# senli1073/SeisT

Measured on NVIDIA H100. Metric: waveforms/sec (B,3,8192) seist_m_dpk fwd+bwd, higher is better.
Workload: dtype f32

## Files before the change

### seist_b200/csrc/api.cu

```cuda
#include <atomic>
#include <cstdio>
#include <cstdlib>
#include <cstring>
#include <vector>
#include "common.cuh"

namespace seist {

static thread_local char g_err[512] = "";
static std::atomic<uint64_t> g_launches{0};
static int g_sm_count = 0;

void set_error(const char* msg) {
  std::strncpy(g_err, msg, sizeof(g_err) - 1);
  g_err[sizeof(g_err) - 1] = 0;
}
void note_launch() { g_launches.fetch_add(1, std::memory_order_relaxed); }
int check_launch(const char* what) {
  cudaError_t e = cudaPeekAtLastError();
  if (e != cudaSuccess) {
    cudaGetLastError();
    std::snprintf(g_err, sizeof(g_err), "%s: %s", what, cudaGetErrorString(e));
    return (int)e;
  }
  return 0;
}

int launch_conv_fwd(const SeistOp& op, cudaStream_t s);
int launch_conv_bwd_data(const SeistOp& op, cudaStream_t s);
int launch_conv_bwd_w(const SeistOp& op, cudaStream_t s, int sm_count);
int launch_res_bwd(const SeistOp& op, cudaStream_t s);
int launch_att_fwd(const SeistOp& op, cudaStream_t s);
int launch_att_bwd_q(const SeistOp& op, cudaStream_t s);
int launch_att_bwd_kv(const SeistOp& op, cudaStream_t s);
int launch_headvec_fwd(const SeistOp& op, cudaStream_t s);
int launch_headvec_bwd(const SeistOp& op, cudaStream_t s);
int launch_bn_finalize(const SeistOp& op, bool fwd, cudaStream_t s);
bool pw_eligible(const SeistOp& op);
int launch_pw_fwd(const SeistOp& op, cudaStream_t s, int sm_count);
int launch_pw_bwd_data(const SeistOp& op, cudaStream_t s, int sm_count);
int launch_res_bwd4(const SeistOp& op, cudaStream_t s, int sm_count);
bool bww_eligible(const SeistOp& op);
int launch_bww_any(const SeistOp& op, cudaStream_t s, int sm_count);
bool convk_eligible(const SeistOp& op);
bool bwwk_eligible(const SeistOp& op);
bool convk_bwd_data_eligible(const SeistOp& op);
int launch_bwwk(const SeistOp& op, cudaStream_t s, int sm_count);
int launch_convk_fwd(const SeistOp& op, cudaStream_t s);
int launch_convk_bwd_data(const SeistOp& op, cudaStream_t s);
int launch_bn_prepare(const SeistOp& op, bool fwd, cudaStream_t s);
int launch_stem_compose(const SeistOp& op, bool fwd, cudaStream_t s);
bool tcconv_eligible(const SeistOp& op, int mode);
int launch_tcconv(const SeistOp& op, int mode, cudaStream_t s, int sm_count);
int tcconv_error_flag();

static int tcc_mode() {
  static int v = -1;
  if (v < 0) { const char* e = std::getenv("SEIST_TCC"); v = !e ? 2 : (e[0] == '0' ? 0 : (e[0] == '1' ? 1 : 2)); }
  return v;
}
static bool tcc_auto(const SeistOp& op, int mode) {
  const int Kd = mode == 0 ? op.Cin : op.Cout;
  if (op.up_src_L > 0) return mode == 0 && Kd >= 32;
  if (op.k > 1) return mode == 0 ? (op.L_out <= 512 && Kd >= 16) : (op.L_out <= 256 && Kd >= 32);
  return mode == 0 && Kd >= 64 && op.L_out <= 256;
}
static bool use_tcc(const SeistOp& op, int mode) {
  const int m = tcc_mode();
  if (m == 0 || !tcconv_eligible(op, mode)) return false;
  return m == 1 || tcc_auto(op, mode);
}

static int sm_count() {
  if (g_sm_count == 0) {
    int dev = 0;
    cudaGetDevice(&dev);
    if (cudaDeviceGetAttribute(&g_sm_count, cudaDevAttrMultiProcessorCount, dev) != cudaSuccess || g_sm_count <= 0)
      g_sm_count = 132;
  }
  return g_sm_count;
}

static int validate_conv(const SeistOp& op) {
  if (op.groups <= 0 || op.Cin % op.groups || op.Cout % op.groups) { set_error("conv: channels not divisible by groups"); return -2; }
  if (op.k < 1 || op.stride < 1 || op.N < 1 || op.L_out < 1) { set_error("conv: bad geometry"); return -2; }
  if (op.n_in < 1 || op.n_in > SEIST_MAX_IN) { set_error("conv: bad n_in"); return -2; }
  if ((op.pool > 1 || op.up_src_L > 0) && op.n_in != 1) { set_error("conv: pool/upsample need a single input view"); return -2; }
  if (op.pool > 1 && (op.k != 1 || op.up_src_L > 0)) { set_error("conv: pool only with k=1"); return -2; }
  if (op.N > 65535) { set_error("conv: batch > 65535 per launch"); return -2; }
  return 0;
}

enum Family {
  F_NONE = 0, F_TCCONV_FWD, F_TCCONV_BWD_DATA, F_PW_FWD, F_CONVK_FWD, F_CONV_FWD, F_PW_BWD_DATA, F_CONVK_BWD_DATA,
  F_CONV_BWD_DATA, F_BWWK, F_BWW, F_CONV_BWD_W, F_RES_BWD, F_RES_BWD4, F_ATT_FWD, F_ATT_BWD_Q, F_ATT_BWD_KV, F_HEADVEC_FWD,
  F_HEADVEC_BWD, F_BN_FINALIZE_FWD, F_BN_FINALIZE_BWD, F_BN_PREPARE_FWD, F_BN_PREPARE_BWD, F_STEM_COMPOSE_FWD, F_STEM_COMPOSE_BWD,
  F_ZERO
};
static const char* kFamilyName[] = {
  "none", "tcconv_fwd(wgmma+TMA)", "tcconv_bwd_data(wgmma+TMA)", "pw_fwd(simt)", "convk_fwd(simt)",
  "conv_fwd(simt)", "pw_bwd_data(simt)", "convk_bwd_data(simt)", "conv_bwd_data(simt)", "bwwk(simt)", "bww(simt)",
  "conv_bwd_w(simt)", "res_bwd", "res_bwd4", "att_fwd", "att_bwd_q", "att_bwd_kv", "headvec_fwd", "headvec_bwd", "bn_finalize_fwd",
  "bn_finalize_bwd", "bn_prepare_fwd", "bn_prepare_bwd", "stem_compose_fwd", "stem_compose_bwd", "zero"
};

static Family choose(const SeistOp& op) {
  switch (op.kind) {
    case SEIST_OP_CONV_FWD:
      if (use_tcc(op, 0)) return F_TCCONV_FWD;
      if (pw_eligible(op)) return F_PW_FWD;
      return convk_eligible(op) ? F_CONVK_FWD : F_CONV_FWD;
    case SEIST_OP_CONV_BWD_DATA:
      if (use_tcc(op, 1)) return F_TCCONV_BWD_DATA;
      if (pw_eligible(op)) return F_PW_BWD_DATA;
      return convk_bwd_data_eligible(op) ? F_CONVK_BWD_DATA : F_CONV_BWD_DATA;
    case SEIST_OP_CONV_BWD_W:
      if (bwwk_eligible(op)) return F_BWWK;
      return bww_eligible(op) ? F_BWW : F_CONV_BWD_W;
    case SEIST_OP_RES_BWD: return (op.L_out & 3) ? F_RES_BWD : F_RES_BWD4;
    case SEIST_OP_ATT_FWD: return F_ATT_FWD;
    case SEIST_OP_ATT_BWD_Q: return F_ATT_BWD_Q;
    case SEIST_OP_ATT_BWD_KV: return F_ATT_BWD_KV;
    case SEIST_OP_HEADVEC_FWD: return F_HEADVEC_FWD;
    case SEIST_OP_HEADVEC_BWD: return F_HEADVEC_BWD;
    case SEIST_OP_BN_FINALIZE_FWD: return F_BN_FINALIZE_FWD;
    case SEIST_OP_BN_FINALIZE_BWD: return F_BN_FINALIZE_BWD;
    case SEIST_OP_BN_PREPARE_FWD: return F_BN_PREPARE_FWD;
    case SEIST_OP_BN_PREPARE_BWD: return F_BN_PREPARE_BWD;
    case SEIST_OP_STEM_COMPOSE_FWD: return F_STEM_COMPOSE_FWD;
    case SEIST_OP_STEM_COMPOSE_BWD: return F_STEM_COMPOSE_BWD;
    case SEIST_OP_ZERO: return F_ZERO;
    default: return F_NONE;
  }
}

static int run_one(const SeistOp& op, cudaStream_t s) {
  if (op.kind == SEIST_OP_CONV_FWD || op.kind == SEIST_OP_CONV_BWD_DATA || op.kind == SEIST_OP_CONV_BWD_W) {
    int v = validate_conv(op);
    if (v) return v;
  }
  switch (choose(op)) {
    case F_TCCONV_FWD: return launch_tcconv(op, 0, s, sm_count());
    case F_TCCONV_BWD_DATA: return launch_tcconv(op, 1, s, sm_count());
    case F_PW_FWD: return launch_pw_fwd(op, s, sm_count());
    case F_CONVK_FWD: return launch_convk_fwd(op, s);
    case F_CONV_FWD: return launch_conv_fwd(op, s);
    case F_PW_BWD_DATA: return launch_pw_bwd_data(op, s, sm_count());
    case F_CONVK_BWD_DATA: return launch_convk_bwd_data(op, s);
    case F_CONV_BWD_DATA: return launch_conv_bwd_data(op, s);
    case F_BWWK: return launch_bwwk(op, s, sm_count());
    case F_BWW: return launch_bww_any(op, s, sm_count());
    case F_CONV_BWD_W: return launch_conv_bwd_w(op, s, sm_count());
    case F_RES_BWD: return launch_res_bwd(op, s);
    case F_RES_BWD4: return launch_res_bwd4(op, s, sm_count());
    case F_ATT_FWD: return launch_att_fwd(op, s);
    case F_ATT_BWD_Q: return launch_att_bwd_q(op, s);
    case F_ATT_BWD_KV: return launch_att_bwd_kv(op, s);
    case F_HEADVEC_FWD: return launch_headvec_fwd(op, s);
    case F_HEADVEC_BWD: return launch_headvec_bwd(op, s);
    case F_BN_FINALIZE_FWD: return launch_bn_finalize(op, true, s);
    case F_BN_FINALIZE_BWD: return launch_bn_finalize(op, false, s);
    case F_BN_PREPARE_FWD: return launch_bn_prepare(op, true, s);
    case F_BN_PREPARE_BWD: return launch_bn_prepare(op, false, s);
    case F_STEM_COMPOSE_FWD: return launch_stem_compose(op, true, s);
    case F_STEM_COMPOSE_BWD: return launch_stem_compose(op, false, s);
    case F_ZERO: {
      cudaError_t e = cudaMemsetAsync(op.out.x, 0, op.zero_bytes, s);
      if (e != cudaSuccess) { set_error(cudaGetErrorString(e)); return (int)e; }
      return 0;
    }
    default: set_error("unknown op kind"); return -1;
  }
}

}

extern "C" {

int seist_plan_run(const SeistOp* ops, int32_t n, void* stream);
const char* seist_last_error(void);

int seist_abi_version(void) { return SEIST_ABI_VERSION; }
uint64_t seist_sizeof_op(void) { return sizeof(SeistOp); }
uint64_t seist_sizeof_bn(void) { return sizeof(SeistBN); }
const char* seist_last_error(void) { return seist::g_err; }
uint64_t seist_launch_count(void) { return seist::g_launches.load(); }
const char* seist_op_family(const SeistOp* op) { return op ? seist::kFamilyName[seist::choose(*op)] : "none"; }
int seist_tc_error_flag(void) { return seist::tcconv_error_flag(); }

static std::vector<cudaEvent_t> g_events[64];
static cudaEvent_t event_at(size_t i) {
  int dev = 0;
  cudaGetDevice(&dev);
  std::vector<cudaEvent_t>& pool = g_events[dev & 63];
  while (pool.size() <= i) {
    cudaEvent_t e = nullptr;
    if (cudaEventCreateWithFlags(&e, cudaEventDisableTiming) != cudaSuccess) return nullptr;
    pool.push_back(e);
  }
  return pool[i];
}
static int fork_join(cudaStream_t from, cudaStream_t to, size_t& ev) {
  cudaEvent_t e = event_at(ev++);
  if (e == nullptr) { seist::set_error("plan_run_lanes: cudaEventCreate failed"); return (int)cudaErrorMemoryAllocation; }
  cudaError_t r = cudaEventRecord(e, from);
  if (r == cudaSuccess) r = cudaStreamWaitEvent(to, e, 0);
  if (r != cudaSuccess) { seist::set_error(cudaGetErrorString(r)); return (int)r; }
  return 0;
}

int seist_plan_run_lanes(const SeistOp* ops, int32_t n, void* const* streams, int32_t n_streams) {
  if (ops == nullptr || n < 0 || streams == nullptr || n_streams < 1 || n_streams > 8) { seist::set_error("plan_run_lanes: bad arguments"); return -1; }
  if (n_streams == 1) return seist_plan_run(ops, n, streams[0]);
  cudaStream_t s0 = (cudaStream_t)streams[0];
  size_t ev = (size_t)n;
  for (int l = 1; l < n_streams; ++l) {
    size_t e = ev;
    const int fr = fork_join(s0, (cudaStream_t)streams[l], e);
    if (fr) return fr;
  }
  int rc = 0;
  for (int i = 0; i < n && rc == 0; ++i) {
    const SeistOp& op = ops[i];
    const int lane = op.lane < 0 ? 0 : (op.lane >= n_streams ? n_streams - 1 : op.lane);
    cudaStream_t s = (cudaStream_t)streams[lane];
    for (int w = 0; w < op.n_wait && w < 4 && rc == 0; ++w) {
      if (op.wait_ev[w] < 0 || op.wait_ev[w] >= n) { seist::set_error("plan_run_lanes: bad event id"); rc = -1; break; }
      cudaEvent_t e = event_at((size_t)op.wait_ev[w]);
      cudaError_t r = e ? cudaStreamWaitEvent(s, e, 0) : cudaErrorMemoryAllocation;
      if (r != cudaSuccess) { seist::set_error(cudaGetErrorString(r)); rc = (int)r; }
    }
    if (rc) break;
    rc = seist::run_one(op, s);
    if (rc != 0) {
      char buf[600];
      std::snprintf(buf, sizeof(buf), "op %d (kind %d): %s", i, op.kind, seist_last_error());
      seist::set_error(buf);
      break;
    }
    if (op.rec_event >= 0) {
      cudaEvent_t e = op.rec_event < n ? event_at((size_t)op.rec_event) : nullptr;
      cudaError_t r = e ? cudaEventRecord(e, s) : cudaErrorMemoryAllocation;
      if (r != cudaSuccess) { seist::set_error(cudaGetErrorString(r)); rc = (int)r; }
    }
  }
  for (int l = 1; l < n_streams; ++l) {
    size_t e = (size_t)n + 1 + (size_t)l;
    const int jr = fork_join((cudaStream_t)streams[l], s0, e);
    if (jr && !rc) rc = jr;
  }
  return rc;
}

int seist_plan_run(const SeistOp* ops, int32_t n, void* stream) {
  if (ops == nullptr || n < 0) { seist::set_error("plan_run: bad arguments"); return -1; }
  cudaStream_t s = (cudaStream_t)stream;
  for (int i = 0; i < n; ++i) {
    int rc = seist::run_one(ops[i], s);
    if (rc != 0) {
      char buf[600];
      std::snprintf(buf, sizeof(buf), "op %d (kind %d): %s", i, ops[i].kind, seist::g_err);
      seist::set_error(buf);
      return rc;
    }
  }
  return 0;
}

}
```

### seist_b200/csrc/pw.cu

```cuda
#include "common.cuh"
#include "conv_common.cuh"

namespace seist {

constexpr int PW_NT = 128;

__device__ __forceinline__ float4 ldg4(const float* p) { return __ldg(reinterpret_cast<const float4*>(p)); }
__device__ __forceinline__ float4 ld4(const float* p) { return *reinterpret_cast<const float4*>(p); }
__device__ __forceinline__ void st4(float* p, float4 v) { *reinterpret_cast<float4*>(p) = v; }

__device__ __forceinline__ float4 lds4(uint32_t a) {
  float4 v;
  asm volatile("ld.shared.v4.f32 {%0,%1,%2,%3}, [%4];" : "=f"(v.x), "=f"(v.y), "=f"(v.z), "=f"(v.w) : "r"(a));
  return v;
}

struct PwChan {
  const float* x;
  float* g;
  long long nstride;
  float sc, sh, mu, istd;
  int act, bn, bnc, accum;
};

// ... 406 lines not shown
  if constexpr (RING) {
    iobase = quad_base(0);
#pragma unroll
    for (int s = 0; s < PW_RING_S - 1; ++s) issue_step();
  }

  for (int g = 0; g < G; ++g) {
    const long long f = ((long long)blockIdx.x * G + g) * PW_NT + tid;
    const bool ok = f < NQ;
    const int n = ok ? (int)(f / LQ) : 0;
    const int l = ok ? (int)(f - (long long)n * LQ) * 4 : 0;
    const float pf = path_factor(op, seed, n) * alpha_factor(op, seed, n);
    float2 acc[CI_T / 2][4];
#pragma unroll
    for (int c = 0; c < CI_T / 2; ++c)
#pragma unroll
      for (int q = 0; q < 4; ++q) acc[c][q] = make_float2(0.f, 0.f);
    const size_t obase = ((size_t)n * op.out.Ct + op.out.c0) * (size_t)L + l;
    for (int co0 = 0; co0 < Cout4; co0 += PW_BD_CG) {
      float4 dx[PW_BD_CG], du[PW_BD_CG], xo[PW_BD_CG];
      if constexpr (RING) {
        issue_step();
        cp_async_wait<PW_RING_S - 1>();
        const uint32_t src0 = ring + cstage * PW_RING_STAGE_B;
        cstage = cstage + 1 == PW_RING_S ? 0 : cstage + 1;
#pragma unroll
        for (int j = 0; j < PW_BD_CG; ++j) {
          const uint32_t src = src0 + j * (3 * PW_NT * 16);
          dx[j] = op.out_dxd ? lds4(src) : make_float4(0.f, 0.f, 0.f, 0.f);
          du[j] = has_bn ? lds4(src + PW_NT * 16) : make_float4(0.f, 0.f, 0.f, 0.f);
          xo[j] = need_x ? lds4(src + 2 * PW_NT * 16) : make_float4(0.f, 0.f, 0.f, 0.f);
        }
      } else {
#pragma unroll
        for (int j = 0; j < PW_BD_CG; ++j) {
          const int co = min(co0 + j, Cout - 1);
          const size_t off = obase + (size_t)co * L;
          dx[j] = op.out_dxd ? ldg4(op.out_dxd + off) : make_float4(0.f, 0.f, 0.f, 0.f);
          du[j] = has_bn ? ldg4(op.out.g + off) : make_float4(0.f, 0.f, 0.f, 0.f);
          xo[j] = need_x ? ldg4(op.out.x + off) : make_float4(0.f, 0.f, 0.f, 0.f);
        }
      }
#pragma unroll
      for (int j = 0; j < PW_BD_CG; ++j) {
        const int co = co0 + j;
        const PwOut o = oc_s[co];
        float4 gv;
        gv.x = dx[j].x + fmaf(o.A, du[j].x, fmaf(o.Bx, xo[j].x, o.Cc));
        gv.y = dx[j].y + fmaf(o.A, du[j].y, fmaf(o.Bx, xo[j].y, o.Cc));
        gv.z = dx[j].z + fmaf(o.A, du[j].z, fmaf(o.Bx, xo[j].z, o.Cc));
        gv.w = dx[j].w + fmaf(o.A, du[j].w, fmaf(o.Bx, xo[j].w, o.Cc));
        if (op.out_act == SEIST_OUT_SIGMOID) {
          gv.x *= xo[j].x * (1.f - xo[j].x);
          gv.y *= xo[j].y * (1.f - xo[j].y);
          gv.z *= xo[j].z * (1.f - xo[j].z);
          gv.w *= xo[j].w * (1.f - xo[j].w);
        }
        gv.x *= pf;
        gv.y *= pf;
        gv.z *= pf;
        gv.w *= pf;
        if (F_ELEM) {
          const float4 kp = pw_keep4(op.p_elem, seed, op.seed_elem, ((uint64_t)n * Cout + min(co, Cout - 1)) * (uint64_t)L + l);
          gv.x *= kp.x;
          gv.y *= kp.y;
          gv.z *= kp.z;
          gv.w *= kp.w;
        }
        const float2* wr = reinterpret_cast<const float2*>(w_s + co * CI_T);
        const float2 gx = dup2(gv.x), gy = dup2(gv.y), gz = dup2(gv.z), gw = dup2(gv.w);
#pragma unroll
        for (int cp = 0; cp < CI_T / 2; ++cp) {
          const float2 w = wr[cp];
          acc[cp][0] = fma2(w, gx, acc[cp][0]);
          acc[cp][1] = fma2(w, gy, acc[cp][1]);
          acc[cp][2] = fma2(w, gz, acc[cp][2]);
          acc[cp][3] = fma2(w, gw, acc[cp][3]);
        }
      }
    }
    if (!ok) continue;
    if constexpr (F_POOL) {
#pragma unroll
      for (int col = 0; col < CI_T; ++col) {
        const PwChan& c = ch_s[col];
        if (c.g == nullptr) continue;
        const float2(&ap)[4] = acc[col >> 1];
        float4 gg = (col & 1) ? make_float4(ap[0].y, ap[1].y, ap[2].y, ap[3].y) : make_float4(ap[0].x, ap[1].x, ap[2].x, ap[3].x);
        {
          const long long soff = (long long)n * c.nstride + (long long)l * op.pool;
          float s1 = 0.f, s2 = 0.f;
          if (op.pool == 2) pool_route<2>(c, soff, gg, s1, s2);
          else if (op.pool == 4) pool_route<4>(c, soff, gg, s1, s2);
          else pool_route<8>(c, soff, gg, s1, s2);
          if (c.bn >= 0) {
            my_st[(2 * col) * 32] += s1;
            my_st[(2 * col + 1) * 32] += s2;
          }
        }
      }
    } else {
#pragma unroll
    for (int cb = 0; cb < CI_T; cb += PW_BD_EB) {
      float4 xv[PW_BD_EB], ov[PW_BD_EB];
#pragma unroll
      for (int u = 0; u < PW_BD_EB; ++u) {
        const PwChan& c = ch_s[cb + u];
        const long long off = (long long)n * c.nstride + l;
        const bool live = c.g != nullptr;
        const bool want_x = live && ((F_GELU && c.act == SEIST_ACT_GELU) || c.bn >= 0);
        xv[u] = want_x ? ldg4(c.x + off) : make_float4(0.f, 0.f, 0.f, 0.f);
        ov[u] = (live && c.accum) ? ld4(c.g + off) : make_float4(0.f, 0.f, 0.f, 0.f);
      }
#pragma unroll
      for (int u = 0; u < PW_BD_EB; ++u) {
        const int col = cb + u;
        const PwChan& c = ch_s[col];
        if (c.g == nullptr) continue;
        const float2(&ap)[4] = acc[col >> 1];
        float4 gg = (col & 1) ? make_float4(ap[0].y, ap[1].y, ap[2].y, ap[3].y) : make_float4(ap[0].x, ap[1].x, ap[2].x, ap[3].x);
        const float4 x = xv[u];
        if (F_GELU && c.act == SEIST_ACT_GELU) {
          const float4 d = pw_gelu_grad4(make_float4(fmaf(c.sc, x.x, c.sh), fmaf(c.sc, x.y, c.sh), fmaf(c.sc, x.z, c.sh),
                                                     fmaf(c.sc, x.w, c.sh)));
          gg.x *= d.x;
          gg.y *= d.y;
          gg.z *= d.z;
          gg.w *= d.w;
        }
        if (c.bn >= 0) {
          my_st[(2 * col) * 32] += (gg.x + gg.y) + (gg.z + gg.w);
          my_st[(2 * col + 1) * 32] += fmaf(gg.x, (x.x - c.mu) * c.istd, gg.y * ((x.y - c.mu) * c.istd)) +
                                       fmaf(gg.z, (x.z - c.mu) * c.istd, gg.w * ((x.w - c.mu) * c.istd));
        }
        gg.x += ov[u].x;
        gg.y += ov[u].y;
        gg.z += ov[u].z;
        gg.w += ov[u].w;
        st4(c.g + (long long)n * c.nstride + l, gg);
      }
    }
    }
  }
  float st[2 * CI_T];
#pragma unroll
  for (int i = 0; i < 2 * CI_T; ++i) st[i] = my_st[i * 32];
  cta_reduce_atomic<2 * CI_T>(st, red_s, [&](int i, float s) {
    const PwChan& c = ch_s[i >> 1];
    if (c.g != nullptr && c.bn >= 0) {
      const SeistBN& e = op.bn_table[c.bn];
      atomicAdd(&e.gstat_acc[(i & 1) * e.C + c.bnc], (double)s);
    }
  });
}

__global__ void __launch_bounds__(PW_NT) res_bwd4_kernel(const __grid_constant__ SeistOp op, const int G) {
  __shared__ float red_s[4 * 4];
  const int tid = threadIdx.x;
  const int co = blockIdx.y;
  const int L = op.L_out, LQ = L >> 2;
  const long long NQ = (long long)op.N * LQ;
  const uint64_t seed = load_seed(op.step_seed);
  const OutGradCoef kc = out_grad_coef(op, co);
  const bool has_bn = (op.out.bn >= 0 && op.out.g != nullptr);
  const bool need_x = has_bn || op.out_act == SEIST_OUT_SIGMOID;
  const SeistView& va = op.res_a;
  const SeistView& vb = op.res_b;
  const bool wa = va.C > 0 && va.g != nullptr, wb = vb.C > 0 && vb.g != nullptr;
  float amu = 0.f, aistd = 0.f, bmu = 0.f, bistd = 0.f;
  if (wa && va.bn >= 0) view_khat(op, va, co, amu, aistd);
  if (wb && vb.bn >= 0) view_khat(op, vb, co, bmu, bistd);
  float st[4] = {0.f, 0.f, 0.f, 0.f};
  for (int g = 0; g < G; ++g) {
    const long long f = ((long long)blockIdx.x * G + g) * PW_NT + tid;
    if (f >= NQ) break;
    const int n = (int)(f / LQ);
    const int l = (int)(f - (long long)n * LQ) * 4;
    const size_t off = ((size_t)n * op.out.Ct + op.out.c0 + co) * (size_t)L + l;
    float4 gv = op.out_dxd ? ldg4(op.out_dxd + off) : make_float4(0.f, 0.f, 0.f, 0.f);
    if (need_x) {
      const float4 x = ldg4(op.out.x + off);
      if (has_bn) {
        const float4 du = ldg4(op.out.g + off);
        gv.x += fmaf(kc.A, du.x, fmaf(kc.Bx, x.x, kc.Cc));
        gv.y += fmaf(kc.A, du.y, fmaf(kc.Bx, x.y, kc.Cc));
        gv.z += fmaf(kc.A, du.z, fmaf(kc.Bx, x.z, kc.Cc));
        gv.w += fmaf(kc.A, du.w, fmaf(kc.Bx, x.w, kc.Cc));
      }
      if (op.out_act == SEIST_OUT_SIGMOID) {
        gv.x *= x.x * (1.f - x.x);
        gv.y *= x.y * (1.f - x.y);
        gv.z *= x.z * (1.f - x.z);
        gv.w *= x.w * (1.f - x.w);
      }
    }
#pragma unroll
    for (int which = 0; which < 2; ++which) {
      const SeistView& v = which == 0 ? va : vb;
      if (!(which == 0 ? wa : wb)) continue;
      float4 gg = gv;
      if (which == 0) {
        const float af = alpha_factor(op, seed, n);
        gg.x *= af;
        gg.y *= af;
        gg.z *= af;
        gg.w *= af;
      }
      const size_t voff = ((size_t)n * v.Ct + v.c0 + co) * (size_t)L + l;
      if (v.bn >= 0) {
        const float4 x = ldg4(v.x + voff);
        const float mu = which == 0 ? amu : bmu, is = which == 0 ? aistd : bistd;
        st[2 * which] += (gg.x + gg.y) + (gg.z + gg.w);
        st[2 * which + 1] += fmaf(gg.x, (x.x - mu) * is, gg.y * ((x.y - mu) * is)) +
                             fmaf(gg.z, (x.z - mu) * is, gg.w * ((x.w - mu) * is));
      }
      float* gp = v.g + voff;
      if (v.accum) {
        const float4 old = ld4(gp);
        gg.x += old.x;
        gg.y += old.y;
        gg.z += old.z;
        gg.w += old.w;
      }
      st4(gp, gg);
    }
  }
  cta_reduce_atomic<4>(st, red_s, [&](int i, float s) {
    const SeistView& v = (i >> 1) == 0 ? va : vb;
    const bool w = (i >> 1) == 0 ? wa : wb;
    if (w && v.bn >= 0) {
      const SeistBN& e = op.bn_table[v.bn];
      atomicAdd(&e.gstat_acc[(i & 1) * e.C + v.bn_c0 + co], (double)s);
    }
  });
}

static bool pw_pooled_ok(const SeistOp& op) {
  if (op.pool != 2 && op.pool != 4 && op.pool != 8) return false;
  if (op.n_in != 1 || op.in[0].act != SEIST_ACT_NONE || op.in[0].L != op.L_out * op.pool) return false;
  return op.p_elem <= 0.f && op.res_a.C == 0 && op.res_b.C == 0;
}
bool pw_eligible(const SeistOp& op) {
  if (op.k != 1 || op.stride != 1 || op.groups != 1 || op.up_src_L > 0) return false;
  if (op.L_out & 3) return false;
  if (op.pool > 1) return pw_pooled_ok(op);
  return true;
}

static int pick_G(long long nq, int tiles_y, int sm_count) {
  long long ctas = (nq + PW_NT - 1) / PW_NT;
  int G = 1;
  while (G < 8 && (ctas / (2 * G)) * tiles_y >= 4LL * sm_count) G *= 2;
  return G;
}

template <typename K>
static int pw_set_smem(K kernel, size_t bytes) {
  if (bytes > 48 * 1024) {
    cudaError_t e = cudaFuncSetAttribute(kernel, cudaFuncAttributeMaxDynamicSharedMemorySize, (int)bytes);
    if (e != cudaSuccess) return (int)e;
  }
  return 0;
}

static bool any_gelu(const SeistOp& op) {
  for (int i = 0; i < op.n_in; ++i)
    if (op.in[i].act == SEIST_ACT_GELU) return true;
  return false;
}

template <int COT, bool E, bool R, bool Gf, bool P = false>
static int pw_fwd_go(const SeistOp& op, cudaStream_t s, dim3 grid, size_t smem, int G) {
  int rc = pw_set_smem(pw_fwd_kernel<COT, E, R, Gf, P>, smem);
  if (!rc) pw_fwd_kernel<COT, E, R, Gf, P><<<grid, PW_NT, smem, s>>>(op, G);
  return rc;
}
template <int COT>
static int pw_fwd_sel(const SeistOp& op, cudaStream_t s, dim3 grid, size_t smem, int G) {
  if (op.pool > 1) return pw_fwd_go<COT, false, false, false, true>(op, s, grid, smem, G);
  const int sel = (op.p_elem > 0.f ? 4 : 0) | ((op.res_a.C > 0 || op.res_b.C > 0) ? 2 : 0) | (any_gelu(op) ? 1 : 0);
  switch (sel) {
    case 0: return pw_fwd_go<COT, false, false, false>(op, s, grid, smem, G);
    case 1: return pw_fwd_go<COT, false, false, true>(op, s, grid, smem, G);
    case 2: return pw_fwd_go<COT, false, true, false>(op, s, grid, smem, G);
    case 3: return pw_fwd_go<COT, false, true, true>(op, s, grid, smem, G);
    case 4: return pw_fwd_go<COT, true, false, false>(op, s, grid, smem, G);
    case 5: return pw_fwd_go<COT, true, false, true>(op, s, grid, smem, G);
    case 6: return pw_fwd_go<COT, true, true, false>(op, s, grid, smem, G);
    default: return pw_fwd_go<COT, true, true, true>(op, s, grid, smem, G);
  }
}

int launch_pw_fwd(const SeistOp& op, cudaStream_t s, int sm_count) {
  const int cot = op.Cout > 8 ? 16 : 8;
  const int Cin8 = (op.Cin + 7) & ~7;
  const size_t smem = sizeof(PwChan) * Cin8 + sizeof(float) * ((size_t)Cin8 * cot + 5 * cot + 4 * 2 * cot + 4 * 2 * cot * 32);
  const long long nq = (long long)op.N * (op.L_out >> 2);
  const int ty = (op.Cout + cot - 1) / cot;
  const int G = pick_G(nq, ty, sm_count);
  dim3 grid((unsigned)((nq + (long long)PW_NT * G - 1) / ((long long)PW_NT * G)), ty);
  const int rc = cot == 16 ? pw_fwd_sel<16>(op, s, grid, smem, G) : pw_fwd_sel<8>(op, s, grid, smem, G);
  if (rc) return rc;
  note_launch();
  return check_launch("pw_fwd");
}

template <int CIT, bool E, bool Gf, bool P = false>
static int pw_bwdd_go(const SeistOp& op, cudaStream_t s, dim3 grid, size_t smem, int G) {
  if (!P) smem += (size_t)PW_RING_S * PW_RING_STAGE_B;
  int rc = pw_set_smem(pw_bwd_data_kernel<CIT, E, Gf, P>, smem);
  if (!rc) pw_bwd_data_kernel<CIT, E, Gf, P><<<grid, PW_NT, smem, s>>>(op, G);
  return rc;
}
template <int CIT>
static int pw_bwdd_sel(const SeistOp& op, cudaStream_t s, dim3 grid, size_t smem, int G) {
  if (op.pool > 1) return pw_bwdd_go<CIT, false, false, true>(op, s, grid, smem, G);
  const int sel = (op.p_elem > 0.f ? 2 : 0) | (any_gelu(op) ? 1 : 0);
  switch (sel) {
    case 0: return pw_bwdd_go<CIT, false, false>(op, s, grid, smem, G);
    case 1: return pw_bwdd_go<CIT, false, true>(op, s, grid, smem, G);
    case 2: return pw_bwdd_go<CIT, true, false>(op, s, grid, smem, G);
    default: return pw_bwdd_go<CIT, true, true>(op, s, grid, smem, G);
  }
}

int launch_pw_bwd_data(const SeistOp& op, cudaStream_t s, int sm_count) {
  const int cit = op.Cin > 8 ? 16 : 8;
  const int Cout4 = (op.Cout + 3) & ~3;
  const size_t smem = sizeof(PwChan) * cit + sizeof(PwOut) * Cout4 + sizeof(float) * ((size_t)Cout4 * cit + 4 * 2 * cit + 4 * 2 * cit * 32);
  const long long nq = (long long)op.N * (op.L_out >> 2);
  const int ty = (op.Cin + cit - 1) / cit;
  const int G = pick_G(nq, ty, sm_count);
  dim3 grid((unsigned)((nq + (long long)PW_NT * G - 1) / ((long long)PW_NT * G)), ty);
  const int rc = cit == 16 ? pw_bwdd_sel<16>(op, s, grid, smem, G) : pw_bwdd_sel<8>(op, s, grid, smem, G);
  if (rc) return rc;
  note_launch();
  return check_launch("pw_bwd_data");
}

int launch_res_bwd4(const SeistOp& op, cudaStream_t s, int sm_count) {
  const long long nq = (long long)op.N * (op.L_out >> 2);
  const int G = pick_G(nq, op.Cout, sm_count);
  dim3 grid((unsigned)((nq + (long long)PW_NT * G - 1) / ((long long)PW_NT * G)), op.Cout);
  res_bwd4_kernel<<<grid, PW_NT, 0, s>>>(op, G);
  note_launch();
  return check_launch("res_bwd4");
}

constexpr int BW_NT = 256;

template <int CO_B, int R_B, bool K1, int BW_PC>
__global__ void __launch_bounds__(BW_NT, 3) bww_kernel(const __grid_constant__ SeistOp op, const int nci_max, const int g_async, const int gx_off) {
  constexpr int BW_PITCH = BW_PC + 4;
  constexpr int BW_GP = 2 * BW_PC + 8;
  extern __shared__ __align__(16) unsigned char sm_raw[];
  constexpr int TGM = CO_B / 4, TGN = R_B / 8, TG = TGM * TGN, PG = BW_NT / TG;
  static_assert(TG <= BW_NT && BW_NT % TG == 0, "bad tile");
  const int k = op.k, S = op.stride, L = op.L_out;
  const int gs_in = op.Cin / op.groups, gs_out = op.Cout / op.groups;
  const int tpg = (gs_out + CO_B - 1) / CO_B;
  const int grp = blockIdx.y / tpg;
  const int Cin = (grp + 1) * gs_in;
  const int Cout = (grp + 1) * gs_out;
  const int R = gs_in * k;
  const int width = BW_PC * S + k - S;
  const int pitch = K1 ? BW_PITCH : (width | 1);
  const int stage_f = (CO_B / 2) * BW_GP + nci_max * pitch;
  const int area_f = stage_f > BW_NT * 36 ? stage_f : BW_NT * 36;
  float* g_s = reinterpret_cast<float*>(sm_raw);
  float* in_s = g_s + (CO_B / 2) * BW_GP;
  PwOut* oc_s = reinterpret_cast<PwOut*>(g_s + ((area_f + 3) & ~3));
  PwChan* ch_s = reinterpret_cast<PwChan*>(oc_s + CO_B);
  float* src_s = reinterpret_cast<float*>(ch_s + nci_max + 1);
  float* gx_s = reinterpret_cast<float*>(sm_raw) + gx_off;
  float* gd_s = gx_s + (CO_B / 2) * BW_GP;
  const int tid = threadIdx.x, lane = tid & 31, warp = tid >> 5;
  const int co_base = grp * gs_out + (blockIdx.y - grp * tpg) * CO_B, r_base = blockIdx.z * R_B;
  const int ci_lo = grp * gs_in + r_base / k;
  const int ci_hi = min(grp * gs_in + (r_base + R_B - 1) / k, Cin - 1);
  const int nci = ci_hi - ci_lo + 1;

  for (int col = tid; col < CO_B; col += BW_NT) {
    const int co = co_base + col;
    PwOut o = {0.f, 0.f, 0.f};
    if (co < Cout) {
      const OutGradCoef kc = out_grad_coef(op, co);
      o.A = kc.A;
      o.Bx = kc.Bx;
      o.Cc = kc.Cc;
    }
    oc_s[col] = o;
  }
  if (K1)
    for (int row = tid; row < nci; row += BW_NT) ch_s[row] = make_chan(op, ci_lo + row, false);
  __syncthreads();

  const uint64_t seed = load_seed(op.step_seed);
  const bool has_bn = (op.out.bn >= 0 && op.out.g != nullptr);
  const bool need_x = has_bn || op.out_act == SEIST_OUT_SIGMOID;
  const bool vec = (L & 3) == 0;
  const bool plain = op.pool <= 1 && op.up_src_L == 0;
  const int Lsrc = op.in[0].L;
  const float ratio = op.up_src_L > 0 ? (float)Lsrc / (float)op.L_in : 1.f;
  const int tcoord = tid % TG, pg = tid / TG;
  const int tm = tcoord / TGN, tn = tcoord % TGN;
  int roff[8];
#pragma unroll
  for (int j = 0; j < 8; ++j) {
    const int r = r_base + tn + TGN * j;
    const int rr = r < R ? r : r_base;
    const int q = rr / k, t = rr - q * k;
    roff[j] = (grp * gs_in + q - ci_lo) * pitch + t;
  }
  float2 acc[2][8];
  float2 bacc[2] = {make_float2(0.f, 0.f), make_float2(0.f, 0.f)};
#pragma unroll
  for (int i = 0; i < 2; ++i)
#pragma unroll
    for (int j = 0; j < 8; ++j) acc[i][j] = make_float2(0.f, 0.f);

  const int chunks_per_n = (L + BW_PC - 1) / BW_PC;
  const int total = op.N * chunks_per_n;
  constexpr int QPR = BW_PC / 4;
  for (int tile = blockIdx.x; tile < total; tile += gridDim.x) {
    const int n = tile / chunks_per_n;
    const int l0 = (tile - n * chunks_per_n) * BW_PC;
    const float pf = path_factor(op, seed, n) * alpha_factor(op, seed, n);
    const bool in_async = K1 && vec && plain;
    if (in_async) {
      for (int idx = tid; idx < nci * QPR; idx += BW_NT) {
        const int row = idx / QPR, q = idx - row * QPR;
        const int l = l0 + 4 * q;
        float* dst = in_s + row * pitch + 4 * q;
        if (l < L) {
          const PwChan& c = ch_s[row];
          cp_async16(smem_addr(dst), c.x + (long long)n * c.nstride + l);
        } else {
          st4(dst, make_float4(0.f, 0.f, 0.f, 0.f));
        }
      }
      cp_async_commit();
    }
    if (vec && g_async) {
      gacc_issue<BW_NT>(op, n, l0, L, co_base, Cout, CO_B, QPR, BW_GP, g_s, gx_s, gd_s, has_bn, need_x);
      cp_async_commit();
      cp_async_wait<0>();
      gacc_combine<BW_NT>(op, n, l0, L, co_base, Cout, CO_B, QPR, BW_GP, g_s, gx_s, gd_s, oc_s, has_bn, need_x, pf, seed, op.Cout);
    } else if (vec) {
      for (int idx = tid; idx < (CO_B / 2) * QPR; idx += BW_NT) {
        const int pr = idx / QPR, q = idx - pr * QPR;
        const int l = l0 + 4 * q;
        float4 gh[2];
#pragma unroll
        for (int h = 0; h < 2; ++h) {
          const int row = 2 * pr + h, co = co_base + row;
          float4 gv = make_float4(0.f, 0.f, 0.f, 0.f);
          if (co < Cout && l < L) {
            const size_t off = ((size_t)n * op.out.Ct + op.out.c0 + co) * (size_t)L + l;
            if (op.out_dxd) gv = ldg4(op.out_dxd + off);
            if (need_x) {
              const float4 x = ldg4(op.out.x + off);
              if (has_bn) {
                const float4 du = ldg4(op.out.g + off);
                const PwOut o = oc_s[row];
                gv = add4(gv, fma4(splat4(o.A), du, fma4(splat4(o.Bx), x, splat4(o.Cc))));
              }
              if (op.out_act == SEIST_OUT_SIGMOID) gv = mul4(gv, mul4(x, fma4(x, splat4(-1.f), splat4(1.f))));
            }
            gv = scale4(gv, pf);
            if (op.p_elem > 0.f) gv = mul4(gv, keep4(op.p_elem, seed, op.seed_elem, ((uint64_t)n * Cout + co) * (uint64_t)L + l));
          }
          gh[h] = gv;
        }
        float* gp = g_s + pr * BW_GP + 8 * q;
        st4(gp, make_float4(gh[0].x, gh[1].x, gh[0].y, gh[1].y));
        st4(gp + 4, make_float4(gh[0].z, gh[1].z, gh[0].w, gh[1].w));
      }
    } else {
      for (int idx = tid; idx < CO_B * BW_PC; idx += BW_NT) {
        const int row = idx / BW_PC, pos = idx - row * BW_PC;
        const int co = co_base + row, l = l0 + pos;
        float v = 0.f;
        if (co < Cout && l < L) {
          OutGradCoef kc;
          kc.A = oc_s[row].A;
          kc.Bx = oc_s[row].Bx;
          kc.Cc = oc_s[row].Cc;
          v = out_grad_at(op, kc, n, co, l) * pf * elem_factor(op, seed, n, co, l);
        }
        g_s[(row >> 1) * BW_GP + 2 * pos + (row & 1)] = v;
      }
    }
// ... 186 lines not shown
```

Measured before the change: 9412.

## Add cp.async-staged persistent pointwise backward-data kernel for mid-size Cin

Adds a new persistent kernel for pointwise conv backward-data with Cin between 17 and 192. Output-gradient inputs are streamed through a 3-stage cp.async shared-memory ring in chunks of 8 output channels, and each warp computes 16 input channels with packed float2 FMAs. BN gradient statistics are reduced by warp butterfly halving and written with one atomic per warp at the end. The aim is to overlap global loads with compute and to reuse staged gradients across all input channels instead of recomputing per tile. The cost is large shared-memory use for the full weight matrix and block-wide syncs on every chunk.

```diff
diff --git a/seist_b200/csrc/api.cu b/seist_b200/csrc/api.cu
--- a/seist_b200/csrc/api.cu
+++ b/seist_b200/csrc/api.cu
@@ -39,6 +39,8 @@
 bool pw_eligible(const SeistOp& op);
 int launch_pw_fwd(const SeistOp& op, cudaStream_t s, int sm_count);
 int launch_pw_bwd_data(const SeistOp& op, cudaStream_t s, int sm_count);
+bool pw_bwd_data_staged_ok(const SeistOp& op);
+int launch_pw_bwd_data_staged(const SeistOp& op, cudaStream_t s, int sm_count);
 int launch_res_bwd4(const SeistOp& op, cudaStream_t s, int sm_count);
 bool bww_eligible(const SeistOp& op);
 int launch_bww_any(const SeistOp& op, cudaStream_t s, int sm_count);
@@ -92,14 +94,14 @@
 }
 
 enum Family {
-  F_NONE = 0, F_TCCONV_FWD, F_TCCONV_BWD_DATA, F_PW_FWD, F_CONVK_FWD, F_CONV_FWD, F_PW_BWD_DATA, F_CONVK_BWD_DATA,
+  F_NONE = 0, F_TCCONV_FWD, F_TCCONV_BWD_DATA, F_PW_FWD, F_CONVK_FWD, F_CONV_FWD, F_PW_BWD_DATA, F_PW_BWD_DATA_STAGED, F_CONVK_BWD_DATA,
   F_CONV_BWD_DATA, F_BWWK, F_BWW, F_CONV_BWD_W, F_RES_BWD, F_RES_BWD4, F_ATT_FWD, F_ATT_BWD_Q, F_ATT_BWD_KV, F_HEADVEC_FWD,
   F_HEADVEC_BWD, F_BN_FINALIZE_FWD, F_BN_FINALIZE_BWD, F_BN_PREPARE_FWD, F_BN_PREPARE_BWD, F_STEM_COMPOSE_FWD, F_STEM_COMPOSE_BWD,
   F_ZERO
 };
 static const char* kFamilyName[] = {
   "none", "tcconv_fwd(wgmma+TMA)", "tcconv_bwd_data(wgmma+TMA)", "pw_fwd(simt)", "convk_fwd(simt)",
-  "conv_fwd(simt)", "pw_bwd_data(simt)", "convk_bwd_data(simt)", "conv_bwd_data(simt)", "bwwk(simt)", "bww(simt)",
+  "conv_fwd(simt)", "pw_bwd_data(simt)", "pw_bwd_data_staged(simt)", "convk_bwd_data(simt)", "conv_bwd_data(simt)", "bwwk(simt)", "bww(simt)",
   "conv_bwd_w(simt)", "res_bwd", "res_bwd4", "att_fwd", "att_bwd_q", "att_bwd_kv", "headvec_fwd", "headvec_bwd", "bn_finalize_fwd",
   "bn_finalize_bwd", "bn_prepare_fwd", "bn_prepare_bwd", "stem_compose_fwd", "stem_compose_bwd", "zero"
 };
@@ -112,6 +114,7 @@
       return convk_eligible(op) ? F_CONVK_FWD : F_CONV_FWD;
     case SEIST_OP_CONV_BWD_DATA:
       if (use_tcc(op, 1)) return F_TCCONV_BWD_DATA;
+      if (pw_bwd_data_staged_ok(op)) return F_PW_BWD_DATA_STAGED;
       if (pw_eligible(op)) return F_PW_BWD_DATA;
       return convk_bwd_data_eligible(op) ? F_CONVK_BWD_DATA : F_CONV_BWD_DATA;
     case SEIST_OP_CONV_BWD_W:
@@ -146,6 +149,7 @@
     case F_CONVK_FWD: return launch_convk_fwd(op, s);
     case F_CONV_FWD: return launch_conv_fwd(op, s);
     case F_PW_BWD_DATA: return launch_pw_bwd_data(op, s, sm_count());
+    case F_PW_BWD_DATA_STAGED: return launch_pw_bwd_data_staged(op, s, sm_count());
     case F_CONVK_BWD_DATA: return launch_convk_bwd_data(op, s);
     case F_CONV_BWD_DATA: return launch_conv_bwd_data(op, s);
     case F_BWWK: return launch_bwwk(op, s, sm_count());
diff --git a/seist_b200/csrc/pw.cu b/seist_b200/csrc/pw.cu
--- a/seist_b200/csrc/pw.cu
+++ b/seist_b200/csrc/pw.cu
@@ -582,6 +582,240 @@
       atomicAdd(&e.gstat_acc[(i & 1) * e.C + c.bnc], (double)s);
     }
   });
+}
+
+constexpr int PWS_CC = 8;
+constexpr int PWS_S = 3;
+constexpr int PWS_PLANE_B = 32 * 16;
+constexpr int PWS_STAGE_B = PWS_CC * 3 * PWS_PLANE_B;
+constexpr int PWS_MAX_CIN = 192;
+
+__device__ __forceinline__ void sts4(uint32_t a, float4 v) {
+  asm volatile("st.shared.v4.f32 [%0], {%1,%2,%3,%4};" ::"r"(a), "f"(v.x), "f"(v.y), "f"(v.z), "f"(v.w) : "memory");
+}
+
+template <int H>
+__device__ __forceinline__ void warp_halve(float* v, int lane) {
+  const bool up = (lane & H) != 0;
+#pragma unroll
+  for (int k = 0; k < H; ++k) {
+    const float send = up ? v[k] : v[k + H];
+    const float keep = up ? v[k + H] : v[k];
+    v[k] = keep + __shfl_xor_sync(0xffffffffu, send, H);
+  }
+}
+
+template <bool F_ELEM, bool F_GELU>
+__global__ void __launch_bounds__(PWS_MAX_CIN * 2) pw_bwd_data_staged_kernel(const __grid_constant__ SeistOp op) {
+  extern __shared__ __align__(16) unsigned char sm_raw[];
+  const int NT = blockDim.x, NW = NT >> 5;
+  const int Cout = op.Cout, Cin = op.Cin, Cin16 = NW * 16;
+  const int nck = (Cout + PWS_CC - 1) / PWS_CC, CoutC = nck * PWS_CC;
+  PwChan* ch_s = reinterpret_cast<PwChan*>(sm_raw);
+  PwOut* oc_s = reinterpret_cast<PwOut*>(ch_s + Cin16);
+  float* w_s = reinterpret_cast<float*>(oc_s + CoutC);
+  const uint32_t ring = smem_addr(w_s + CoutC * Cin16);
+  const int tid = threadIdx.x, lane = tid & 31, warp = tid >> 5;
+  const int L = op.L_out, LQ = L >> 2;
+
+  for (int ci = tid; ci < Cin16; ci += NT) {
+    PwChan c = make_chan(op, ci < Cin ? ci : 0, true);
+    if (ci >= Cin) c.g = nullptr;
+    ch_s[ci] = c;
+  }
+  for (int co = tid; co < CoutC; co += NT) {
+    PwOut o = {0.f, 0.f, 0.f};
+    if (co < Cout) {
+      const OutGradCoef k = out_grad_coef(op, co);
+      o.A = k.A;
+      o.Bx = k.Bx;
+      o.Cc = k.Cc;
+    }
+    oc_s[co] = o;
+  }
+  for (int idx = tid; idx < CoutC * Cin16; idx += NT) {
+    const int co = idx / Cin16, ci = idx - co * Cin16;
+    w_s[idx] = (co < Cout && ci < Cin) ? op.W[(size_t)co * Cin + ci] : 0.f;
+  }
+  __syncthreads();
+
+  const uint64_t seed = load_seed(op.step_seed);
+  const long long NQ = (long long)op.N * LQ;
+  const long long ntiles = (NQ + 31) / 32;
+  const bool has_dxd = op.out_dxd != nullptr;
+  const bool has_bn = (op.out.bn >= 0 && op.out.g != nullptr);
+  const bool need_x = has_bn || op.out_act == SEIST_OUT_SIGMOID;
+  auto quad_of = [&](long long tile, int& n, int& l) -> bool {
+    const long long f = tile * 32 + lane;
+    const bool ok = f < NQ;
+    n = ok ? (int)(f / LQ) : 0;
+    l = ok ? (int)(f - (long long)n * LQ) * 4 : 0;
+    return ok;
+  };
+
+  long long itile = blockIdx.x;
+  int ick = 0, istage = 0;
+  int in_, il;
+  bool iok = quad_of(itile, in_, il);
+  size_t iobase = ((size_t)in_ * op.out.Ct + op.out.c0) * (size_t)L + il;
+  auto issue_step = [&]() {
+    if (itile < ntiles) {
+      const uint32_t dst0 = ring + istage * PWS_STAGE_B + lane * 16;
+      for (int c = warp; c < PWS_CC; c += NW) {
+        const int co = ick * PWS_CC + c;
+        if (iok && co < Cout) {
+          const size_t off = iobase + (size_t)co * L;
+          const uint32_t dst = dst0 + c * (3 * PWS_PLANE_B);
+          if (has_dxd) cp_async16(dst, op.out_dxd + off);
+          if (has_bn) cp_async16(dst + PWS_PLANE_B, op.out.g + off);
+          if (need_x) cp_async16(dst + 2 * PWS_PLANE_B, op.out.x + off);
+        }
+      }
+      if (++ick == nck) {
+        ick = 0;
+        itile += gridDim.x;
+        iok = quad_of(itile, in_, il);
+        iobase = ((size_t)in_ * op.out.Ct + op.out.c0) * (size_t)L + il;
+      }
+    }
+    cp_async_commit();
+    istage = istage + 1 == PWS_S ? 0 : istage + 1;
+  };
+#pragma unroll
+  for (int s = 0; s < PWS_S - 1; ++s) issue_step();
+
+  bool warp_bn = false;
+  for (int t = 0; t < 16; ++t) {
+    const PwChan& c = ch_s[warp * 16 + t];
+    warp_bn |= c.g != nullptr && c.bn >= 0;
+  }
+  const PwChan* my_ch = ch_s + warp * 16;
+  float st_run = 0.f;
+  int cstage = 0;
+  for (long long tile = blockIdx.x; tile < ntiles; tile += gridDim.x) {
+    int n, l;
+    const bool ok = quad_of(tile, n, l);
+    const float pf = path_factor(op, seed, n) * alpha_factor(op, seed, n);
+    float2 acc[8][4];
+#pragma unroll
+    for (int c = 0; c < 8; ++c)
+#pragma unroll
+      for (int q = 0; q < 4; ++q) acc[c][q] = make_float2(0.f, 0.f);
+    for (int ck = 0; ck < nck; ++ck) {
+      cp_async_wait<PWS_S - 2>();
+      const uint32_t st = ring + cstage * PWS_STAGE_B + lane * 16;
+      cstage = cstage + 1 == PWS_S ? 0 : cstage + 1;
+      for (int c = warp; c < PWS_CC; c += NW) {
+        const int co = ck * PWS_CC + c;
+        const uint32_t slot = st + c * (3 * PWS_PLANE_B);
+        float4 gv = make_float4(0.f, 0.f, 0.f, 0.f);
+        if (ok && co < Cout) {
+          const float4 dx = has_dxd ? lds4(slot) : make_float4(0.f, 0.f, 0.f, 0.f);
+          const float4 du = has_bn ? lds4(slot + PWS_PLANE_B) : make_float4(0.f, 0.f, 0.f, 0.f);
+          const float4 xo = need_x ? lds4(slot + 2 * PWS_PLANE_B) : make_float4(0.f, 0.f, 0.f, 0.f);
+          const PwOut o = oc_s[co];
+          gv.x = dx.x + fmaf(o.A, du.x, fmaf(o.Bx, xo.x, o.Cc));
+          gv.y = dx.y + fmaf(o.A, du.y, fmaf(o.Bx, xo.y, o.Cc));
+          gv.z = dx.z + fmaf(o.A, du.z, fmaf(o.Bx, xo.z, o.Cc));
+          gv.w = dx.w + fmaf(o.A, du.w, fmaf(o.Bx, xo.w, o.Cc));
+          if (op.out_act == SEIST_OUT_SIGMOID) {
+            gv.x *= xo.x * (1.f - xo.x);
+            gv.y *= xo.y * (1.f - xo.y);
+            gv.z *= xo.z * (1.f - xo.z);
+            gv.w *= xo.w * (1.f - xo.w);
+          }
+          gv.x *= pf;
+          gv.y *= pf;
+          gv.z *= pf;
+          gv.w *= pf;
+          if (F_ELEM) {
+            const float4 kp = pw_keep4(op.p_elem, seed, op.seed_elem, ((uint64_t)n * Cout + co) * (uint64_t)L + l);
+            gv.x *= kp.x;
+            gv.y *= kp.y;
+            gv.z *= kp.z;
+            gv.w *= kp.w;
+          }
+        }
+        sts4(slot, gv);
+      }
+      __syncthreads();
+      issue_step();
+      const float* wr0 = w_s + ck * PWS_CC * Cin16 + warp * 16;
+#pragma unroll
+      for (int c = 0; c < PWS_CC; ++c) {
+        const float4 g = lds4(st + c * (3 * PWS_PLANE_B));
+        const float2* wr = reinterpret_cast<const float2*>(wr0 + c * Cin16);
+        const float2 gx = dup2(g.x), gy = dup2(g.y), gz = dup2(g.z), gw = dup2(g.w);
+#pragma unroll
+        for (int cp = 0; cp < 8; ++cp) {
+          const float2 w = wr[cp];
+          acc[cp][0] = fma2(w, gx, acc[cp][0]);
+          acc[cp][1] = fma2(w, gy, acc[cp][1]);
+          acc[cp][2] = fma2(w, gz, acc[cp][2]);
+          acc[cp][3] = fma2(w, gw, acc[cp][3]);
+        }
+      }
+    }
+    float bs[32];
+#pragma unroll
+    for (int cb = 0; cb < 16; cb += PW_BD_EB) {
+      float4 xv[PW_BD_EB], ov[PW_BD_EB];
+#pragma unroll
+      for (int u = 0; u < PW_BD_EB; ++u) {
+        const PwChan& c = my_ch[cb + u];
+        const long long off = (long long)n * c.nstride + l;
+        const bool live = ok && c.g != nullptr;
+        const bool want_x = live && ((F_GELU && c.act == SEIST_ACT_GELU) || c.bn >= 0);
+        xv[u] = want_x ? ldg4(c.x + off) : make_float4(0.f, 0.f, 0.f, 0.f);
+        ov[u] = (live && c.accum) ? ld4(c.g + off) : make_float4(0.f, 0.f, 0.f, 0.f);
+      }
+#pragma unroll
+      for (int u = 0; u < PW_BD_EB; ++u) {
+        const int col = cb + u;
+        const PwChan& c = my_ch[col];
+        bs[2 * col] = 0.f;
+        bs[2 * col + 1] = 0.f;
+        if (!ok || c.g == nullptr) continue;
+        const float2(&ap)[4] = acc[col >> 1];
+        float4 gg = (col & 1) ? make_float4(ap[0].y, ap[1].y, ap[2].y, ap[3].y) : make_float4(ap[0].x, ap[1].x, ap[2].x, ap[3].x);
+        const float4 x = xv[u];
+        if (F_GELU && c.act == SEIST_ACT_GELU) {
+          const float4 d = pw_gelu_grad4(make_float4(fmaf(c.sc, x.x, c.sh), fmaf(c.sc, x.y, c.sh), fmaf(c.sc, x.z, c.sh),
+                                                     fmaf(c.sc, x.w, c.sh)));
+          gg.x *= d.x;
+          gg.y *= d.y;
+          gg.z *= d.z;
+          gg.w *= d.w;
+        }
+        if (c.bn >= 0) {
+          bs[2 * col] = (gg.x + gg.y) + (gg.z + gg.w);
+          bs[2 * col + 1] = fmaf(gg.x, (x.x - c.mu) * c.istd, gg.y * ((x.y - c.mu) * c.istd)) +
+                            fmaf(gg.z, (x.z - c.mu) * c.istd, gg.w * ((x.w - c.mu) * c.istd));
+        }
+        gg.x += ov[u].x;
+        gg.y += ov[u].y;
+        gg.z += ov[u].z;
+        gg.w += ov[u].w;
+        st4(c.g + (long long)n * c.nstride + l, gg);
+      }
+    }
+    if (warp_bn) {
+      warp_halve<16>(bs, lane);
+      warp_halve<8>(bs, lane);
+      warp_halve<4>(bs, lane);
+      warp_halve<2>(bs, lane);
+      warp_halve<1>(bs, lane);
+      st_run += bs[0];
+    }
+  }
+  cp_async_wait<0>();
+  if (warp_bn) {
+    const PwChan& c = my_ch[lane >> 1];
+    if (c.g != nullptr && c.bn >= 0) {
+      const SeistBN& e = op.bn_table[c.bn];
+      atomicAdd(&e.gstat_acc[(lane & 1) * e.C + c.bnc], (double)st_run);
+    }
+  }
 }
 
 __global__ void __launch_bounds__(PW_NT) res_bwd4_kernel(const __grid_constant__ SeistOp op, const int G) {
@@ -768,6 +1002,51 @@
   return check_launch("pw_bwd_data");
 }
 
+static size_t pw_bwd_data_staged_smem(const SeistOp& op) {
+  const int cin16 = (op.Cin + 15) & ~15, coutc = (op.Cout + PWS_CC - 1) / PWS_CC * PWS_CC;
+  return sizeof(PwChan) * cin16 + sizeof(PwOut) * coutc + sizeof(float) * (size_t)coutc * cin16 + (size_t)PWS_S * PWS_STAGE_B;
+}
+
+bool pw_bwd_data_staged_ok(const SeistOp& op) {
+  return pw_eligible(op) && op.pool <= 1 && op.Cin > 16 && op.Cin <= PWS_MAX_CIN && (op.Cin > 32 || !any_gelu(op)) &&
+         pw_bwd_data_staged_smem(op) <= 227 * 1024;
+}
+
+template <bool E, bool Gf>
+static int pw_bwdd_staged_go(const SeistOp& op, cudaStream_t s, int sm_count) {
+  const auto kernel = pw_bwd_data_staged_kernel<E, Gf>;
+  const size_t smem = pw_bwd_data_staged_smem(op);
+  const int nt = 32 * ((op.Cin + 15) / 16);
+  int rc = pw_set_smem(kernel, smem);
+  if (rc) return rc;
+  int per_sm = 0;
+  const cudaError_t e = cudaOccupancyMaxActiveBlocksPerMultiprocessor(&per_sm, kernel, nt, smem);
+  if (e != cudaSuccess) return (int)e;
+  if (per_sm < 1) {
+    set_error("pw_bwd_data_staged: no resident CTA fits");
+    return -2;
+  }
+  const long long tiles = ((long long)op.N * (op.L_out >> 2) + 31) / 32;
+  const long long resident = (long long)per_sm * sm_count;
+  const long long grid = tiles < resident ? tiles : resident;
+  kernel<<<(unsigned)grid, nt, smem, s>>>(op);
+  return 0;
+}
+
+int launch_pw_bwd_data_staged(const SeistOp& op, cudaStream_t s, int sm_count) {
+  const int sel = (op.p_elem > 0.f ? 2 : 0) | (any_gelu(op) ? 1 : 0);
+  int rc;
+  switch (sel) {
+    case 0: rc = pw_bwdd_staged_go<false, false>(op, s, sm_count); break;
+    case 1: rc = pw_bwdd_staged_go<false, true>(op, s, sm_count); break;
+    case 2: rc = pw_bwdd_staged_go<true, false>(op, s, sm_count); break;
+    default: rc = pw_bwdd_staged_go<true, true>(op, s, sm_count); break;
+  }
+  if (rc) return rc;
+  note_launch();
+  return check_launch("pw_bwd_data_staged");
+}
+
 int launch_res_bwd4(const SeistOp& op, cudaStream_t s, int sm_count) {
   const long long nq = (long long)op.N * (op.L_out >> 2);
   const int G = pick_G(nq, op.Cout, sm_count);
```

New measurement: 9723 (median of 6 runs). 3.3% higher.
